# pkubioinformatics/nanoreviser

Measured on AMD Instinct MI355X. Metric: bases revised/sec (whole node), higher is better.
Workload: dtype f32 via scaled 2xf16 split (f32 accumulate)

## Files before the change

### nanoreviser_amd/csrc/nrv_api.hip

```cpp
#include "../../include/nanorev.h"
#include "nrv_kernels.h"
#include "nrv_tailfit.h"
#include "nrv_block.h"

#include <algorithm>
#include <cmath>
#include <cstdio>
#include <cstdlib>
#include <cstring>
#include <string>
#include <chrono>
#include <vector>

using namespace nrv;

#ifdef NRV_DEV_FAST
#define NRV_ACT1(...)
#else
#define NRV_ACT1(...) __VA_ARGS__
#endif

namespace {

thread_local std::string g_create_error = "";
// ... 689 lines not shown
            if (sc > 0 && sw > 0) { const double l = (room / sc - std::fabs((double)c0u[24 + o])) / sw; if (l < xl) xl = l; }
          }
          e2[24] = (float)(xl > 0 ? xl : 0.0);
        }
        d.cr_ep = put(e2, 25);
        const float* Wd = b.t(32);
        std::vector<uint16_t> df((size_t)13 * 4 * 2 * 512, 0);
        NRV_FOR (int ks = 0; ks < 13; ++ks)
          NRV_FOR (int mt = 0; mt < 4; ++mt)
            NRV_FOR (int lane = 0; lane < 64; ++lane)
              NRV_FOR (int j = 0; j < 8; ++j) {
                const int m = lane & 15, kg = lane >> 4;
                const int pos = 4 * ks + 2 * (j >> 2) + (kg >> 1), ch = 4 * (kg & 1) + (j & 3);
                const float v = pos < 50 ? std::ldexp(Wd[(size_t)(pos * 8 + ch) * 64 + 16 * mt + m], 10) : 0.f;
                const size_t o = ((size_t)((ks * 4 + mt) * 2) * 64 + lane) * 8 + j;
                split_f16(v, &df[o], &df[o + 512]);
              }
        std::vector<float> d2(df.size() / 2);
        memcpy(d2.data(), df.data(), df.size() * 2);
        d.cr_d = put(d2.data(), d2.size());
      }
      const float* c0 = host.data() + d.conv;
      memcpy(d.cr_k.w1, c0, 24 * 4);
      memcpy(d.cr_k.b1, c0 + 24, 8 * 4);
      NRV_FOR (int o = 0; o < 8; ++o) { d.cr_k.s1[o] = std::ldexp(c0[32 + o], 6); d.cr_k.h1[o] = std::ldexp(c0[40 + o], 6); }
    }
    const int K0[4] = {0, 32, 128, 256}, K1[4] = {0, 0, 64, 0}, s0[4] = {0, sX1, sX2, sX3}, s1[4] = {0, 0, sS, 0};
    const std::vector<float>* osc[4] = {nullptr, &sc2, &sc3, nullptr};
    const std::vector<float>* osh[4] = {nullptr, &sh2, &sh3, nullptr};
    const int sout[4] = {0, sX2, sX3, 13};
    d.hsc = pack_head_h2(b, wp, bs);
    d.h_w2 = put(wp.data(), wp.size());
    d.h_b2 = put(bs.data(), bs.size());
    NRV_FOR (int l = 1; l < 4; ++l) {
      const int E = plan_exponent(b, lbase[l], K0[l], s0[l], K1[l], s1[l], lH[l]);
      if (l == 1) {
        pack_lstm2_t(b, lbase[1], sX1, E, wp, bs);
        d.l2t_w = put(wp.data(), wp.size());
        d.l2t_b = put(bs.data(), bs.size());
      }
      if (l >= 2) {
        const int Kf = l == 2 ? 128 : 256;
        const std::vector<float>& fsc = l == 2 ? sc2 : sc3;
        const std::vector<float>& fsh = l == 2 ? sh2 : sh3;
        std::vector<float> all(b.p, b.p + b.off.back() + (size_t)C);
        NRV_FOR (int dir = 0; dir < 2; ++dir) {
          float* W = all.data() + b.off[lbase[l] + dir * 3 + 0];
          float* B = all.data() + b.off[lbase[l] + dir * 3 + 2];
          const int N4 = 4 * lH[l];
          NRV_FOR (int c = 0; c < N4; ++c) {
            double acc = B[c];
            NRV_FOR (int k = 0; k < Kf; ++k) acc += (double)fsh[k] * (double)W[(size_t)k * N4 + c];
            B[c] = (float)acc;
          }
          NRV_FOR (int k = 0; k < Kf; ++k)
            NRV_FOR (int c = 0; c < N4; ++c) W[(size_t)k * N4 + c] *= fsc[k];
        }
        const Blob bf{all.data(), b.off};
        const int Ef = plan_exponent(bf, lbase[l], K0[l], 13, K1[l], s1[l], lH[l]);
        pack_lstm_h2s(bf, lbase[l], K0[l], 13, K1[l], s1[l], lH[l], Ef, wp, bs, kUhS[l]);
        d.l_w2sf[l] = put(wp.data(), wp.size());
        d.l_b2sf[l] = put(bs.data(), bs.size());
        d.descale_f[l] = std::ldexp(1.f, -Ef);
      }
      d.descale[l] = std::ldexp(1.f, -E);
      std::vector<float> one(2 * lH[l], 1.f), zero(2 * lH[l], 0.f);
      d.l_s2[l] = put_scaled(osc[l] ? *osc[l] : one, sout[l] - 13);
      d.l_h2[l] = put_scaled(osh[l] ? *osh[l] : zero, sout[l]);
    }
  }
  pack_lstm1_16(b, 12, wp, bs);
  d.l1w16 = put(wp.data(), wp.size());
  d.l1b16 = put(bs.data(), bs.size());
  pack_dense(b.t(50), 128, 128, wp); d.d1p = put(wp.data(), wp.size());
  d.d1b = put(b.t(51), 128);
  pack_dense(b.t(52), 128, 32, wp); d.d2p = put(wp.data(), wp.size());
  d.d2b = put(b.t(53), 32);
  pack_dense(b.t(54), 32, 6, wp); d.mop = put(wp.data(), wp.size());
  {
    float mb[32] = {0};
    memcpy(mb, b.t(55), 6 * 4);
    d.mob = put(mb, 32);
  }
  pack_head_split(b, wp, bs);
  d.h_ws = put(wp.data(), wp.size());
  d.h_wb = put(bs.data(), bs.size());
  d.fw = put(b.t(56), (size_t)6 * T * 16);
  {
    std::vector<float> f8((size_t)16 * T * 8, 0.f);
    const float* fwp = b.t(56);
    NRV_FOR (int f = 0; f < 16; ++f)
      NRV_FOR (int t = 0; t < T; ++t)
        NRV_FOR (int k = 0; k < 6; ++k) f8[((size_t)f * T + t) * 8 + k] = fwp[(size_t)(t * 6 + k) * 16 + f];
    d.fw8 = put(f8.data(), f8.size());
  }
  d.fb = put(b.t(57), 16);
  d.ow = put(b.t(58), (size_t)16 * C);
  d.ob = put(b.t(59), C);
  d.n = host.size();
  HIPCHK(h, hipMalloc(&d.all, d.n * sizeof(float)));
  HIPCHK(h, hipMemcpy(d.all, host.data(), d.n * sizeof(float), hipMemcpyHostToDevice));
  return NRV_OK;
}

static void free_workspace(nrv_handle* h) {
  for (int m = 0; m < 2; ++m) {
    (void)hipFree(h->S[m]); (void)hipFree(h->X1[m]); (void)hipFree(h->X2[m]); (void)hipFree(h->X3[m]);
    (void)hipFree(h->MO[m]); h->MO[m] = nullptr;
    for (int st = 0; st < 2; ++st) { h->d_p[st][m] = nullptr; h->d_a[st][m] = nullptr; }
    h->S[m] = h->X1[m] = h->X2[m] = h->X3[m] = nullptr;
  }
  for (int st = 0; st < 2; ++st) {
    (void)hipFree(h->d_out[st]);
    h->d_out[st] = nullptr; h->d_sat_st[st] = nullptr; h->pin_sat[st] = nullptr; h->sat_seen[st] = 0;
    (void)hipHostFree(h->pin_out[st]);
    h->pin_out[st] = nullptr;
  }
  for (int st = 0; st < nrv_handle::kIn; ++st) {
    (void)hipFree(h->d_sig[st]); (void)hipFree(h->d_feat[st]);
    h->d_sig[st] = h->d_feat[st] = nullptr;
    (void)hipHostFree(h->pin_sig[st]); (void)hipHostFree(h->pin_feat[st]);
    h->pin_sig[st] = h->pin_feat[st] = nullptr;
  }
  h->pin_sig_cap = h->pin_feat_cap = 0;
  h->cap_rows = 0;
}

constexpr int kCoalesce = 4096;
static int group_windows(const nrv_handle* h) { return (h->coalesce && h->batch < kCoalesce) ? kCoalesce : h->batch; }

static int lanes_wanted(const nrv_handle* h) {
  if (h->coalesce) return 0;
  if (!h->lanes_on || h->batch > 2048 || h->batch % 32) return 0;
  const int w = 4096 / h->batch;
  return w > nrv_handle::kMaxLanes ? nrv_handle::kMaxLanes : w;
}
constexpr int kReadStageGroups = 4;
static int read_stage_groups(const nrv_handle* h) {
  static const int env = getenv("NRV_READ_STAGE") ? atoi(getenv("NRV_READ_STAGE")) : kReadStageGroups;
  return (lanes_wanted(h) > 1 || env < 1) ? 1 : (env > 8 ? 8 : env);
}
static int stage_windows(const nrv_handle* h, bool read_mode = false) {
  const int w = lanes_wanted(h);
  if (w > 1) return w * h->batch;
  return read_mode ? read_stage_groups(h) * group_windows(h) : group_windows(h);
}

static int ensure_workspace(nrv_handle* h) {
  const int T = h->T;
  const int rows = ((stage_windows(h, true) + kRowPad - 1) / kRowPad) * kRowPad;
  if (rows <= h->cap_rows) return NRV_OK;
  free_workspace(h);
  int rc;
  const size_t tiles = (size_t)(((group_windows(h) + kRowPad - 1) / kRowPad) * kRowPad) / 32;
  for (int m = 0; m < 2; ++m) {
    size_t nS = (tiles * T + 2) * 16 * 128, n1 = tiles * T * 8 * 128, n2 = tiles * T * 32 * 128,
           n3 = tiles * T * 64 * 128;
    HIPCHK(h, hipMalloc(&h->S[m], nS * 4));
    HIPCHK(h, hipMalloc(&h->X1[m], n1 * 4));
    HIPCHK(h, hipMalloc(&h->X2[m], n2 * 4));
    HIPCHK(h, hipMalloc(&h->X3[m], n3 * 4));
    HIPCHK(h, hipMalloc(&h->MO[m], tiles * T * 256 * 4));
    const size_t nm = tiles * T * 256;
    if ((rc = alloc_fill(h, h->MO[m], nm * 4)) || (rc = alloc_fill(h, h->S[m], nS * 4)) || (rc = alloc_fill(h, h->X1[m], n1 * 4)) ||
        (rc = alloc_fill(h, h->X2[m], n2 * 4)) || (rc = alloc_fill(h, h->X3[m], n3 * 4)))
      return rc;
    if (m == 0) { h->act_n[0] = nS; h->act_n[1] = n1; h->act_n[2] = n2; h->act_n[3] = n3; h->act_n[4] = nm; }
  }
  h->sig_bytes = (size_t)rows * T * kSig * 4 + 4096;
  h->feat_bytes = (size_t)rows * T * kFeat * 4 + 4096;
  for (int st = 0; st < nrv_handle::kIn; ++st) {
    HIPCHK(h, hipMalloc(&h->d_sig[st], h->sig_bytes));
    HIPCHK(h, hipMalloc(&h->d_feat[st], h->feat_bytes));
    if ((rc = poison_fill(h, h->d_sig[st], h->sig_bytes, nullptr)) || (rc = poison_fill(h, h->d_feat[st], h->feat_bytes, nullptr)))
      return rc;
  }
  for (int st = 0; st < 2; ++st) {
    const size_t ob = (size_t)rows * kOutBytes;
    HIPCHK(h, hipMalloc((void**)&h->d_out[st], ob + 64));
    HIPCHK(h, hipMemset(h->d_out[st], 0, ob + 64));
    if ((rc = poison_fill(h, h->d_out[st] + 64, ob, nullptr))) return rc;
    HIPCHK(h, hipHostMalloc((void**)&h->pin_out[st], ob + 64, hipHostMallocDefault));
    memset(h->pin_out[st], 0, ob + 64);
    h->d_p[st][0] = (float*)(h->d_out[st] + 64);
    h->d_p[st][1] = (float*)(h->d_out[st] + 64 + (size_t)rows * 24);
    h->d_a[st][0] = (int8_t*)(h->d_out[st] + 64 + (size_t)rows * 44);
    h->d_a[st][1] = (int8_t*)(h->d_out[st] + 64 + (size_t)rows * 45);
    h->d_sat_st[st] = (unsigned*)h->d_out[st];
    h->pin_sat[st] = (unsigned*)h->pin_out[st];
    h->sat_seen[st] = 0;
  }
  if (h->poison_on) HIPCHK(h, hipDeviceSynchronize());
  h->cap_rows = rows;
  return NRV_OK;
}

static void free_lanes(nrv_handle* h) {
  for (int l = 0; l < nrv_handle::kMaxLanes; ++l) {
    nrv_handle::Lane& L = h->lanes[l];
    if (L.stream) (void)hipStreamSynchronize(L.stream);
    for (int m = 0; m < 2; ++m) {
      (void)hipFree(L.S[m]); (void)hipFree(L.X1[m]); (void)hipFree(L.X2[m]); (void)hipFree(L.X3[m]); (void)hipFree(L.MO[m]);
      L.S[m] = L.X1[m] = L.X2[m] = L.X3[m] = L.MO[m] = nullptr;
    }
  }
  h->n_lanes = 0;
  h->lane_rows = 0;
}

static int ensure_lanes(nrv_handle* h) {
  const int T = h->T;
  const int rows = ((h->batch + kRowPad - 1) / kRowPad) * kRowPad;
  const int want = lanes_wanted(h);
  if (want == h->n_lanes && (want == 0 || rows <= h->lane_rows)) return NRV_OK;
  free_lanes(h);
  if (want == 0) return NRV_OK;
  const size_t tiles = rows / 32;
  const size_t nS = (tiles * T + 2) * 16 * 128, n1 = tiles * T * 8 * 128, n2 = tiles * T * 32 * 128,
               n3 = tiles * T * 64 * 128, nm = tiles * T * 256;
  if (!h->ev_fork) HIPCHK(h, hipEventCreateWithFlags(&h->ev_fork, hipEventDisableTiming));
  for (int l = 0; l < want; ++l) {
    nrv_handle::Lane& L = h->lanes[l];
    if (!L.stream) HIPCHK(h, hipStreamCreateWithFlags(&L.stream, hipStreamNonBlocking));
    if (!L.done) HIPCHK(h, hipEventCreateWithFlags(&L.done, hipEventDisableTiming));
    for (int m = 0; m < 2; ++m) {
      float** bufs[5] = {&L.S[m], &L.X1[m], &L.X2[m], &L.X3[m], &L.MO[m]};
      const size_t sz[5] = {nS, n1, n2, n3, nm};
      for (int i = 0; i < 5; ++i) {
        HIPCHK(h, hipMalloc(bufs[i], sz[i] * 4));
        const int rc = alloc_fill(h, *bufs[i], sz[i] * 4);
        if (rc) return rc;
        L.act_n[i] = sz[i];
      }
    }
  }
  HIPCHK(h, hipDeviceSynchronize());
  h->n_lanes = want;
  h->lane_rows = rows;
  return NRV_OK;
}

template <int KQ0, int KQ1, int H, int R, int WR>
static void launch_lstm_f32(nrv_handle* h, const LstmArgs& a, int tiles) {
  constexpr int NG = (H + 31) / 32;
  static_assert(NG * WR <= 4, "at most 4 waves per workgroup (one per SIMD, 512 registers each)");
#ifdef NRV_DEV_FAST
  return;
#else
  LstmArgs la = a;
  la.n_blk = (tiles + R * WR - 1) / (R * WR);
  dim3 grid(lstm_grid(la.n_blk)), blk(64 * NG * WR);
  if (h->act == 0) hipLaunchKernelGGL((lstm_layer_kernel<KQ0, KQ1, H, R, WR, false, 0>), grid, blk, 0, h->stream, la);
  NRV_ACT1(else hipLaunchKernelGGL((lstm_layer_kernel<KQ0, KQ1, H, R, WR, false, 1>), grid, blk, 0, h->stream, la);)
#endif
}


template <int KQ0, int KQ1, int H, int R, int WR>
static void launch_lstm_split(nrv_handle* h, const LstmArgs& a, const float* const ws[2], int tiles) {
  constexpr int NG = (H + 31) / 32;
#ifdef NRV_DEV_FAST
  return;
#else
  LstmSplitArgs sa;
  sa.T = a.T; sa.n_rows = a.n_rows;
  for (int m = 0; m < 2; ++m)
    sa.m[m] = LstmSplitModelParams{ws[m], a.m[m].bias, a.m[m].bn_scale, a.m[m].bn_shift, a.m[m].in0, a.m[m].in1,
                                   a.m[m].out};
  sa.n_blk = (tiles + R * WR - 1) / (R * WR);
  dim3 grid(lstm_grid(sa.n_blk)), blk(64 * NG * WR);
  if constexpr (R == 1) {
    {
      if (h->act == 0) hipLaunchKernelGGL((lstm_pair_kernel<KQ0, KQ1, H, R, WR, 0>), grid, blk, 0, h->stream, sa);
      NRV_ACT1(else hipLaunchKernelGGL((lstm_pair_kernel<KQ0, KQ1, H, R, WR, 1>), grid, blk, 0, h->stream, sa);)
      return;
    }
  }
  if constexpr (R != 1)
  {
    if (h->act == 0) hipLaunchKernelGGL((lstm_split_kernel<KQ0, KQ1, H, R, WR, 0>), grid, blk, 0, h->stream, sa);
    NRV_ACT1(else hipLaunchKernelGGL((lstm_split_kernel<KQ0, KQ1, H, R, WR, 1>), grid, blk, 0, h->stream, sa);)
  }
#endif
}

template <int KQ0, int KQ1, int H, int R, int WR, int UH, int NBG, int NA, int KBL = 0, bool RAW = false>
static void launch_lstm_h2s(nrv_handle* h, int layer, const ActView (&in0)[2], const ActView (&in1)[2],
                            float* const out[2], int T, int n, int tiles) {
  constexpr int NG = H / (16 * UH);
  LstmH2Args sa;
  sa.T = T; sa.n_rows = n;
  for (int m = 0; m < 2; ++m) {
    const DevModel& d = h->dm[m];
    sa.m[m] = LstmH2ModelParams{d.all + d.l_w2sf[layer], d.all + d.l_b2sf[layer],
                                d.all + d.l_s2[layer], d.all + d.l_h2[layer], in0[m], in1[m], out[m],
                                d.descale_f[layer]};
  }
  sa.n_blk = (tiles + R * WR - 1) / (R * WR);
  dim3 grid(lstm_grid(sa.n_blk)), blk(64 * NG * WR);
  if (h->act == 0) hipLaunchKernelGGL((lstm_h2s_kernel<KQ0, KQ1, H, R, WR, UH, 0, NBG, NA, KBL, RAW>), grid, blk, 0, h->stream, sa);
  NRV_ACT1(else hipLaunchKernelGGL((lstm_h2s_kernel<KQ0, KQ1, H, R, WR, UH, 1, NBG, NA, KBL, RAW>), grid, blk, 0, h->stream, sa);)
}

#ifndef NRV_L3_WS_NBG
#define NRV_L3_WS_NBG 4
#endif
template <int KQ0, int KQ1, int H>
static void launch_lstm_h2w(nrv_handle* h, int layer, const ActView (&in0)[2], const ActView (&in1)[2],
                            float* const out[2], int T, int n, int tiles) {
  LstmH2Args sa;
  sa.T = T; sa.n_rows = n;
  for (int m = 0; m < 2; ++m) {
    const DevModel& d = h->dm[m];
    sa.m[m] = LstmH2ModelParams{d.all + d.l_w2sf[layer], d.all + d.l_b2sf[layer], d.all + d.l_s2[layer], d.all + d.l_h2[layer],
                                in0[m], in1[m], out[m], d.descale_f[layer]};
  }
  sa.n_blk = (tiles + 1) / 2;
  dim3 grid(lstm_grid(sa.n_blk)), blk(512);
  if (h->act == 0) hipLaunchKernelGGL((lstm_h2w_kernel<KQ0, KQ1, H, 0, NRV_L3_WS_NBG>), grid, blk, 0, h->stream, sa);
  NRV_ACT1(else hipLaunchKernelGGL((lstm_h2w_kernel<KQ0, KQ1, H, 1, NRV_L3_WS_NBG>), grid, blk, 0, h->stream, sa);)
}

#if NRV_STAMP
static int g_only_stage = -1;
#define NRV_RUN_STAGE(k) (g_only_stage < 0 || g_only_stage == (k))
#else
#define NRV_RUN_STAGE(k) true
#endif

static int run_group(nrv_handle* h, const float* d_sig, const float* d_feat, int n, bool read_mode,
                     float* d_p1, float* d_p2, int8_t* d_a1, int8_t* d_a2, unsigned* sat) {
  const int T = h->T;
  const int tiles = (n + 31) / 32;
  if (h->poison_on) {
    for (int m = 0; m < 2; ++m) {
      float* const bufs[5] = {h->S[m], h->X1[m], h->X2[m], h->X3[m], h->MO[m]};
      for (int i = 0; i < 5; ++i) {
        const int rc0 = poison_fill(h, bufs[i], h->act_n[i] * 4, h->stream);
        if (rc0) return rc0;
      }
    }
  }
  hipEvent_t* ev = nullptr;
  if (h->prof && (h->prof != 3 || (h->prof_tick++ & 7) == 0)) {
    if (h->ev_used + NRV_N_KERNELS + 1 > h->ev_pool.size()) {
      for (int i = 0; i < NRV_N_KERNELS + 1; ++i) {
        hipEvent_t e;
        HIPCHK(h, hipEventCreate(&e));
        h->ev_pool.push_back(e);
      }
    }
    ev = h->ev_pool.data() + h->ev_used;
    h->ev_used += NRV_N_KERNELS + 1;
    if (h->prof == 1) HIPCHK(h, hipEventRecord(ev[0], h->stream));
  }
  auto mark = [&](int k) -> int {
    if (ev && (h->prof == 1 || k == 3 || k == 4)) HIPCHK(h, hipEventRecord(ev[k], h->stream));
    return NRV_OK;
  };
  int rc;

  bool h2_fused_l1 = false;
  {
    const int n_rows = read_mode ? n + T - 1 : n, Tc = read_mode ? 1 : T;
    const int n_tiles = read_mode ? (n + T - 1 + 31) / 32 : tiles * T;
    const int blocks = n_tiles < 128 ? n_tiles : 128;
    if (h->h2) {
      CnnRArgs a2;
      for (int m = 0; m < 2; ++m) {
        const DevModel& d = h->dm[m];
        a2.m[m] = CnnRModelParams{d.all + d.cr_w2, d.all + d.cr_ep, d.all + d.cr_d, d.all + d.cr_dbias, h->S[m]};
        a2.k[m] = d.cr_k;
      }
      a2.signal = d_sig; a2.T = Tc; a2.n_rows = n_rows; a2.n_tiles = n_tiles; a2.sat = sat;
      a2.l1_T = T; a2.l1_rows = n;
      for (int m = 0; m < 2; ++m) {
        const DevModel& d = h->dm[m];
        a2.l1[m] = Lstm1ModelParams{d.all + d.l1w16, d.all + d.l1b16, d.all + d.l1s2, d.all + d.l1h2, d_feat,
                                    read_mode ? 1 : 0, h->X1[m]};
      }
      const int wg_c = (2 * n_tiles + kCnnRWaves - 1) / kCnnRWaves, wg_l = (2 * ((n + 15) / 16) + kCnnRL1Waves - 1) / kCnnRL1Waves;
      const int wg = wg_c > wg_l ? wg_c : wg_l;
      if (!NRV_RUN_STAGE(0)) {}
      else if (h->act == 0) hipLaunchKernelGGL(cnn_r_kernel<0>, dim3(wg < 128 ? wg : 128, 2), dim3(kCnnRThreads), 0, h->stream, a2);
      NRV_ACT1(else hipLaunchKernelGGL(cnn_r_kernel<1>, dim3(wg < 128 ? wg : 128, 2), dim3(kCnnRThreads), 0, h->stream, a2);)
      h2_fused_l1 = true;
    } else {
      CnnArgs a;
      for (int m = 0; m < 2; ++m) {
        const DevModel& d = h->dm[m];
        a.m[m] = CnnModelParams{d.all + d.conv, d.all + d.dpack, d.all + d.dbias, d.all + d.dsplit, h->S[m]};
      }
      a.signal = d_sig; a.T = Tc; a.n_rows = n_rows; a.n_tiles = n_tiles;
#ifndef NRV_DEV_FAST
      if (h->split & 32) hipLaunchKernelGGL(cnn_kernel<true>, dim3(blocks, 2), dim3(kCnnThreads), 0, h->stream, a);
      else hipLaunchKernelGGL(cnn_kernel<false>, dim3(blocks, 2), dim3(kCnnThreads), 0, h->stream, a);
#endif
    }
    if ((rc = mark(1))) return rc;
  }
  auto win_view = [&](const float* p, int kq) { return ActView{p, kq, 0, T, 1}; };
  {
    LstmArgs a;
    a.T = T; a.n_rows = n;
    if (!h2_fused_l1) {
      Lstm1Args a1;
      a1.T = T; a1.n_rows = n;
      for (int m = 0; m < 2; ++m) {
        const DevModel& d = h->dm[m];
        a1.m[m] = Lstm1ModelParams{d.all + d.l1w16, d.all + d.l1b16, d.all + (h->h2 ? d.l1s2 : d.l_s[0]),
                                   d.all + (h->h2 ? d.l1h2 : d.l_h[0]), d_feat, read_mode ? 1 : 0, h->X1[m]};
      }
      dim3 grid((n + 63) / 64, 2, 2);
      if (h->h2) {
        if (h->act == 0) hipLaunchKernelGGL((lstm1_kernel<0, true>), grid, dim3(256), 0, h->stream, a1);
        NRV_ACT1(else hipLaunchKernelGGL((lstm1_kernel<1, true>), grid, dim3(256), 0, h->stream, a1);)
      } else if (h->act == 0) hipLaunchKernelGGL(lstm1_kernel<0>, grid, dim3(256), 0, h->stream, a1);
      NRV_ACT1(else hipLaunchKernelGGL(lstm1_kernel<1>, grid, dim3(256), 0, h->stream, a1);)
    }
    if ((rc = mark(2))) return rc;
    for (int m = 0; m < 2; ++m) {
      const DevModel& d = h->dm[m];
      a.m[m] = LstmModelParams{d.all + d.l_w[1], d.all + d.l_b[1], d.all + d.l_s[1], d.all + d.l_h[1],
                               win_view(h->X1[m], 8), ActView{}, nullptr, 0, h->X2[m]};
    }
    const ActView none[2] = {ActView{}, ActView{}};
    if (h->h2) {
      Lstm2RArgs ta;
      ta.T = T; ta.n_rows = n;
      for (int m = 0; m < 2; ++m) {
        const DevModel& d = h->dm[m];
        ta.m[m] = Lstm2RModelParams{d.all + d.l2t_w, d.all + d.l2t_b, h->X1[m], h->X2[m], d.descale[1]};
      }
      dim3 grid(2 * ((n + 63) / 64), 2, 2);
      if (!NRV_RUN_STAGE(2)) {}
      else if (h->act == 0) hipLaunchKernelGGL(lstm2_r_kernel<0>, grid, dim3(kL2rThreads), 0, h->stream, ta);
      NRV_ACT1(else hipLaunchKernelGGL(lstm2_r_kernel<1>, grid, dim3(kL2rThreads), 0, h->stream, ta);)
    }
    else if (h->split & 2) {
      const float* ws[2] = {h->dm[0].all + h->dm[0].l_ws[1], h->dm[1].all + h->dm[1].l_ws[1]};
      launch_lstm_split<8, 0, 64, 1, 2>(h, a, ws, tiles);
    } else {
      launch_lstm_f32<8, 0, 64, 1, 2>(h, a, tiles);
    }
    if ((rc = mark(3))) return rc;
    for (int m = 0; m < 2; ++m) {
      const DevModel& d = h->dm[m];
      ActView sv = read_mode ? ActView{h->S[m], 16, 1, 1, 0} : win_view(h->S[m], 16);
      a.m[m] = LstmModelParams{d.all + d.l_w[2], d.all + d.l_b[2], d.all + d.l_s[2], d.all + d.l_h[2],
                               win_view(h->X2[m], 32), sv, nullptr, 0, h->X3[m]};
    }
    if (h->h2) {
      const ActView i0[2] = {win_view(h->X2[0], 32), win_view(h->X2[1], 32)};
      const ActView i1[2] = {read_mode ? ActView{h->S[0], 16, 1, 1, 0} : win_view(h->S[0], 16),
                             read_mode ? ActView{h->S[1], 16, 1, 1, 0} : win_view(h->S[1], 16)};
      float* const o[2] = {h->X3[0], h->X3[1]};
      if (NRV_RUN_STAGE(3)) launch_lstm_h2w<32, 16, 128>(h, 2, i0, i1, o, T, n, tiles);
    } else if (h->split & 4) {
      const float* ws[2] = {h->dm[0].all + h->dm[0].l_ws[2], h->dm[1].all + h->dm[1].l_ws[2]};
      launch_lstm_split<32, 16, 128, 2, 1>(h, a, ws, tiles);
    } else {
      launch_lstm_f32<32, 16, 128, 1, 1>(h, a, tiles);
    }
    if ((rc = mark(4))) return rc;
    for (int m = 0; m < 2; ++m) {
      const DevModel& d = h->dm[m];
      a.m[m] = LstmModelParams{d.all + d.l_w[3], d.all + d.l_b[3], d.all + d.l_s[3], d.all + d.l_h[3],
                               win_view(h->X3[m], 64), ActView{}, nullptr, 0, h->X2[m] };
    }
    if (h->h2) {
      const ActView i0[2] = {win_view(h->X3[0], 64), win_view(h->X3[1], 64)};
      float* const o[2] = {h->X2[0], h->X2[1]};
      if (NRV_RUN_STAGE(4)) launch_lstm_h2s<64, 0, 64, 2, 1, 1, 8, 2, 3, true>(h, 3, i0, none, o, T, n, tiles);
    } else if (h->split & 8) {
      const float* ws[2] = {h->dm[0].all + h->dm[0].l_ws[3], h->dm[1].all + h->dm[1].l_ws[3]};
      launch_lstm_split<64, 0, 64, 1, 2>(h, a, ws, tiles);
    } else {
      launch_lstm_f32<64, 0, 64, 1, 2>(h, a, tiles);
    }
    if ((rc = mark(5))) return rc;
  }
  {
    float* dp[2] = {d_p1 ? d_p1 : h->d_p[0][0], d_p2 ? d_p2 : h->d_p[0][1]};
    int8_t* da[2] = {d_a1 ? d_a1 : h->d_a[0][0], d_a2 ? d_a2 : h->d_a[0][1]};
    if (h->h2) {
      HeadH2Args ha;
      ha.T = T; ha.n_rows = n; ha.n_tiles = tiles;
      for (int m = 0; m < 2; ++m) {
        const DevModel& d = h->dm[m];
        ha.m[m] = HeadH2ModelParams{d.all + d.h_w2, d.all + d.h_b2, h->X2[m], d.all + d.fw8, d.all + d.fb, d.all + d.ow,
                                    d.all + d.ob, dp[m], da[m], d.hsc.c12, d.hsc.c23, d.hsc.c3o, d.C};
      }
      if (NRV_RUN_STAGE(5)) hipLaunchKernelGGL(head_h2_kernel, dim3(tiles < 128 ? tiles : 128, 2), dim3(kHeadH2Threads), 0, h->stream, ha);
      if ((rc = mark(6))) return rc;
      HIPCHK(h, hipGetLastError());
      return NRV_OK;
    }
    HeadArgs a;
    a.T = T; a.n_rows = n;
    for (int m = 0; m < 2; ++m) {
      const DevModel& d = h->dm[m];
      a.m[m] = HeadModelParams{d.all + d.d1p, d.all + d.d1b, d.all + d.d2p, d.all + d.d2b,
                               d.all + d.mop, d.all + d.mob, d.all + d.fw, d.all + d.fb,
                               d.all + d.ow, d.all + d.ob, h->X2[m], h->MO[m], dp[m], da[m], d.C};
    }
    if (h->split & 16) {
      HeadSplitArgs sa;
      sa.n_units = tiles * T;
      for (int m = 0; m < 2; ++m) {
        const DevModel& d = h->dm[m];
        sa.m[m] = HeadSplitModelParams{d.all + d.h_ws, d.all + d.h_wb, h->X2[m], h->MO[m]};
      }
      const int blocks = sa.n_units < 512 ? (sa.n_units + 3) / 4 : 128;
#ifndef NRV_DEV_FAST
      hipLaunchKernelGGL(head_mlp_split_kernel, dim3(blocks, 2), dim3(256), 0, h->stream, sa);
    } else {
      hipLaunchKernelGGL(head_mlp_kernel, dim3(tiles * T, 2), dim3(64), 0, h->stream, a);
#endif
    }
#ifndef NRV_DEV_FAST
    hipLaunchKernelGGL(head_final_kernel, dim3(tiles, 2), dim3(256), 0, h->stream, a);
#endif
    if ((rc = mark(6))) return rc;
  }
  HIPCHK(h, hipGetLastError());
  return NRV_OK;
}

static int prof_collect(nrv_handle* h) {
  if (h->ev_used == 0) return NRV_OK;
  HIPCHK(h, hipStreamSynchronize(h->stream));
  for (size_t g = 0; g + NRV_N_KERNELS + 1 <= h->ev_used; g += NRV_N_KERNELS + 1)
    for (int k = 0; k < NRV_N_KERNELS; ++k) {
      if (h->prof != 1 && k != 3) continue;
      float ms = 0.f;
      HIPCHK(h, hipEventElapsedTime(&ms, h->ev_pool[g + k], h->ev_pool[g + k + 1]));
      h->prof_ms[k] += ms;
      h->prof_n[k] += 1;
    }
  h->ev_used = 0;
  return NRV_OK;
}

static int check_handle(nrv_handle* h) {
  if (!h) return NRV_E_INVALID;
  hipError_t e = hipSetDevice(h->device);
  if (e != hipSuccess) { h->err = std::string("hipSetDevice: ") + hipGetErrorString(e); return NRV_E_HIP; }
  return NRV_OK;
}

}

extern "C" {

int nrv_create(const nrv_weights* m1, const nrv_weights* m2, int T, int device, int recurrent_act,
               nrv_handle** out) {
  if (!out) { g_create_error = "nrv_create: out is NULL"; return NRV_E_INVALID; }
  *out = nullptr;
  if (T < 1 || T > kMaxT) { g_create_error = "nrv_create: window length T out of range [1,32]"; return NRV_E_INVALID; }
  if (recurrent_act != 0 && recurrent_act != 1) { g_create_error = "nrv_create: recurrent_act must be 0 or 1"; return NRV_E_INVALID; }
  Blob b1, b2;
  if (!make_blob(m1, T, 6, &b1)) { g_create_error = "nrv_create: model1 blob size does not match the graph for this T (expect 6 classes)"; return NRV_E_WEIGHTS; }
  if (!make_blob(m2, T, 5, &b2)) { g_create_error = "nrv_create: model2 blob size does not match the graph for this T (expect 5 classes)"; return NRV_E_WEIGHTS; }
  int ndev = 0;
  hipError_t e = hipGetDeviceCount(&ndev);
  if (e != hipSuccess || ndev <= 0) {
    g_create_error = std::string("nrv_create: no HIP device (") + hipGetErrorString(e) + "); this library has no CPU fallback";
    return NRV_E_NO_DEVICE;
  }
  if (device < 0 || device >= ndev) { g_create_error = "nrv_create: device index out of range"; return NRV_E_NO_DEVICE; }
  e = hipSetDevice(device);
  if (e != hipSuccess) { g_create_error = std::string("hipSetDevice: ") + hipGetErrorString(e); return NRV_E_HIP; }
  nrv_handle* h = new (std::nothrow) nrv_handle();
  if (!h) { g_create_error = "out of host memory"; return NRV_E_NOMEM; }
  h->device = device; h->T = T; h->act = recurrent_act;
  if (const char* s = getenv("NRV_PRECISION")) {
    if (!strcmp(s, "f32")) { h->split = 0; h->h2 = 0; }
    else if (!strcmp(s, "bf16x3")) { h->split = 62; h->h2 = 0; }
    else if (!strcmp(s, "f16x2")) { h->split = 62; h->h2 = 1; }
  }
  int rc = NRV_OK;
  e = hipStreamCreateWithFlags(&h->own_stream, hipStreamDefault);
  if (e != hipSuccess) { g_create_error = std::string("hipStreamCreate: ") + hipGetErrorString(e); delete h; return NRV_E_HIP; }
  h->stream = h->own_stream;
  bool ok = hipStreamCreateWithFlags(&h->copy_stream, hipStreamNonBlocking) == hipSuccess &&
            hipStreamCreateWithFlags(&h->d2h_stream, hipStreamNonBlocking) == hipSuccess;
  for (int st = 0; st < nrv_handle::kIn && ok; ++st) ok = hipEventCreateWithFlags(&h->ev_in[st], hipEventDisableTiming) == hipSuccess;
  for (int st = 0; st < 2 && ok; ++st)
    ok = hipEventCreateWithFlags(&h->ev_done[st], hipEventDisableTiming) == hipSuccess &&
         hipEventCreateWithFlags(&h->ev_out[st], hipEventDisableTiming) == hipSuccess;
  if (const char* e2 = getenv("NRV_HOST_REGISTER")) h->host_register = atoi(e2) != 0;
  if (const char* e3 = getenv("NRV_LANES")) h->lanes_on = atoi(e3) != 0;
  if (const char* e4 = getenv("NRV_COALESCE")) h->coalesce = atoi(e4) != 0;
  if (const char* e6 = getenv("NRV_LABELS_BUDGET"); e6 && *e6) { const long long v = atoll(e6); if (v > 0) h->lab_budget = (size_t)v; }
  if (const char* e7 = getenv("NRV_FIT_MAX_ROWS"); e7 && *e7) { const long long v = atoll(e7); if (v > 0) h->fit.max_rows = v > ((long long)1 << 31) - 1 ? ((long long)1 << 31) - 1 : v; }
  if (const char* e5 = getenv("NRV_POISON"); e5 && *e5) { h->poison_on = true; h->poison = (unsigned)strtoul(e5, nullptr, 16); }
  ok = ok && hipMalloc((void**)&h->d_sat, 4 * sizeof(unsigned)) == hipSuccess &&
       hipMemset(h->d_sat, 0, 4 * sizeof(unsigned)) == hipSuccess;
  if (!ok) { g_create_error = "nrv_create: could not create the copy stream / events / counters"; nrv_destroy(h); return NRV_E_HIP; }
  if ((rc = upload_model(h, 0, b1, 6)) || (rc = upload_model(h, 1, b2, 5)) || (rc = ensure_workspace(h))) {
    g_create_error = h->err;
    nrv_destroy(h);
    return rc;
  }
  *out = h;
  return NRV_OK;
}

void nrv_destroy(nrv_handle* h) {
  if (!h) return;
  (void)hipSetDevice(h->device);
  if (h->stream) (void)hipStreamSynchronize(h->stream);
  free_workspace(h);
  free_lanes(h);
  for (int l = 0; l < nrv_handle::kMaxLanes; ++l) {
    if (h->lanes[l].done) (void)hipEventDestroy(h->lanes[l].done);
    if (h->lanes[l].stream) (void)hipStreamDestroy(h->lanes[l].stream);
  }
  if (h->ev_fork) (void)hipEventDestroy(h->ev_fork);
  for (int m = 0; m < 2; ++m) (void)hipFree(h->dm[m].all);
  for (hipEvent_t e : h->ev_pool) (void)hipEventDestroy(e);
  if (h->copy_stream) { (void)hipStreamSynchronize(h->copy_stream); (void)hipStreamDestroy(h->copy_stream); }
  if (h->d2h_stream) { (void)hipStreamSynchronize(h->d2h_stream); (void)hipStreamDestroy(h->d2h_stream); }
  if (h->edit_stream) { (void)hipStreamSynchronize(h->edit_stream); (void)hipStreamDestroy(h->edit_stream); }
  if (h->lab_stream) { (void)hipStreamSynchronize(h->lab_stream); (void)hipStreamDestroy(h->lab_stream); }
  (void)hipFree(h->d_lab);
  for (char* p : h->lab_retired) (void)hipFree(p);
  for (int m = 0; m < 2; ++m) {
    (void)hipFree(h->fit.flat[m]); (void)hipFree(h->fit.y[m]);
    (void)hipFree(h->fit.m[m].d_par); (void)hipFree(h->fit.m[m].d_state); (void)hipFree(h->fit.m[m].d_lr);
  }
  (void)hipFree(h->fit.d_partial); (void)hipFree(h->fit.d_pstat); (void)hipFree(h->fit.d_order); (void)hipFree(h->fit.d_p);
  for (int st = 0; st < nrv_handle::kIn; ++st) if (h->ev_in[st]) (void)hipEventDestroy(h->ev_in[st]);
  for (int st = 0; st < 2; ++st) {
    if (h->ev_done[st]) (void)hipEventDestroy(h->ev_done[st]);
    if (h->ev_out[st]) (void)hipEventDestroy(h->ev_out[st]);
  }
  (void)hipFree(h->d_raw); (void)hipFree(h->d_starts); (void)hipFree(h->d_reads);
  for (auto& sl : h->raw_slot) {
    (void)hipFree(sl.d_in); (void)hipFree(sl.d_out); (void)hipHostFree(sl.pin_in); (void)hipHostFree(sl.pin_out);
    (void)hipFree(sl.d_stat);
    (void)hipFree(sl.d_mrg); (void)hipHostFree(sl.pin_mrg);
    if (sl.ev_in) (void)hipEventDestroy(sl.ev_in);
    if (sl.ev_done) (void)hipEventDestroy(sl.ev_done);
    if (sl.ev_out) (void)hipEventDestroy(sl.ev_out);
  }
  (void)hipFree(h->d_sat);
  if (h->ev_raw) (void)hipEventDestroy(h->ev_raw);
  if (h->own_stream) (void)hipStreamDestroy(h->own_stream);
  delete h;
}

int nrv_set_batch(nrv_handle* h, int batch) {
  int rc = check_handle(h);
  if (rc) return rc;
  if (batch < 1 || batch > (1 << 20)) { h->err = "nrv_set_batch: batch out of range"; return NRV_E_INVALID; }
  HIPCHK(h, hipStreamSynchronize(h->stream));
  h->batch = batch;
  if ((rc = ensure_workspace(h))) return rc;
  return ensure_lanes(h);
}
int nrv_get_batch(nrv_handle* h) { return h ? h->batch : NRV_E_INVALID; }

int nrv_set_precision(nrv_handle* h, int mode) {
  int rc = check_handle(h);
  if (rc) return rc;
  if (mode != NRV_PREC_F32 && mode != NRV_PREC_BF16X3 && mode != NRV_PREC_F16X2) {
    h->err = "nrv_set_precision: unknown mode";
    return NRV_E_INVALID;
  }
  h->split = mode == NRV_PREC_F32 ? 0 : 62;
  h->h2 = mode == NRV_PREC_F16X2;
  return NRV_OK;
}
int nrv_get_precision(nrv_handle* h) {
  if (!h) return NRV_E_INVALID;
  return h->h2 ? NRV_PREC_F16X2 : (h->split ? NRV_PREC_BF16X3 : NRV_PREC_F32);
}

int nrv_set_stream(nrv_handle* h, void* s) {
  int rc = check_handle(h);
  if (rc) return rc;
  HIPCHK(h, hipStreamSynchronize(h->stream));
  h->stream = s ? (hipStream_t)s : h->own_stream;
  return NRV_OK;
}

int nrv_sync(nrv_handle* h) {
  int rc = check_handle(h);
  if (rc) return rc;
  HIPCHK(h, hipStreamSynchronize(h->stream));
  return NRV_OK;
}

}

template <class F>
static int for_groups(nrv_handle* h, int64_t n, F&& body) {
  const int64_t G = group_windows(h);
  const int64_t ng = (n + G - 1) / G;
  int nl = (h->n_lanes > 1 && ng > 1 && h->prof == 0) ? h->n_lanes : 0;
  if ((int64_t)nl > ng) nl = (int)ng;
  hipStream_t main = h->stream;
  float* keep[5][2];
  for (int m = 0; m < 2; ++m) { keep[0][m] = h->S[m]; keep[1][m] = h->X1[m]; keep[2][m] = h->X2[m]; keep[3][m] = h->X3[m]; keep[4][m] = h->MO[m]; }
  size_t keep_n[5];
  memcpy(keep_n, h->act_n, sizeof keep_n);
  auto restore = [&]() {
    for (int m = 0; m < 2; ++m) { h->S[m] = keep[0][m]; h->X1[m] = keep[1][m]; h->X2[m] = keep[2][m]; h->X3[m] = keep[3][m]; h->MO[m] = keep[4][m]; }
    memcpy(h->act_n, keep_n, sizeof keep_n);
    h->stream = main;
  };
  if (nl) {
    HIPCHK(h, hipEventRecord(h->ev_fork, main));
    for (int l = 0; l < nl; ++l) HIPCHK(h, hipStreamWaitEvent(h->lanes[l].stream, h->ev_fork, 0));
  }
  int rc = NRV_OK;
  int64_t g = 0;
  for (int64_t s = 0; s < n && !rc; s += G, ++g) {
    const int nb = (int)((n - s < G) ? (n - s) : G);
    if (nl) {
      const nrv_handle::Lane& L = h->lanes[g % nl];
      for (int m = 0; m < 2; ++m) { h->S[m] = L.S[m]; h->X1[m] = L.X1[m]; h->X2[m] = L.X2[m]; h->X3[m] = L.X3[m]; h->MO[m] = L.MO[m]; }
      memcpy(h->act_n, L.act_n, sizeof L.act_n);
      h->stream = L.stream;
    }
    rc = body(s, nb);
  }
  restore();
  if (nl) {
    for (int l = 0; l < nl; ++l) {
      hipError_t e = hipEventRecord(h->lanes[l].done, h->lanes[l].stream);
      if (e == hipSuccess) e = hipStreamWaitEvent(main, h->lanes[l].done, 0);
      if (e != hipSuccess && !rc) { h->err = std::string("lane join: ") + hipGetErrorString(e); rc = NRV_E_HIP; }
    }
  }
  return rc;
}

template <class Begin>
static int begin_then_end(nrv_handle* h, Begin begin) {
  int t = -1;
  const int rc = begin(&t);
  return rc ? rc : nrv_reads_raw_end(h, t);
}
template <class Fetch>
static int merged_collect(nrv_handle* h, const char* who, const char* who_edits, const char* head, const MergeView& v,
                          const MergeLayout& m, const MergeOut& o, bool want_q, size_t blob_cap, Fetch fetch) {
  const int64_t n = v.N - h->T > 0 ? v.N - h->T : 0;
  const size_t nb = ((size_t)v.n_reads + 1) * 8;
  const int64_t total = ((const int64_t*)head)[v.n_reads];
  if (total < 0 || total > v.N + n) { h->err = std::string(who) + ": merged block out of range"; return NRV_E_HIP; }
  memcpy(o.off, head, nb);
  if (o.seq) memcpy(o.seq, head + m.seq, (size_t)total);
  if (want_q && o.qual) memcpy(o.qual, head + m.qual, (size_t)total);
  if (o.report) memcpy(o.report, head + m.rep, (size_t)v.n_reads * kReportCols * 8);
  if (o.profile) memcpy(o.profile, head + m.prof, (size_t)v.n_reads * kProfileCols * 8);
  if (o.trim) memcpy(o.trim, head + m.trim, (size_t)v.n_reads * 16);
  if (o.accuracy) memcpy(o.accuracy, head + m.accu, (size_t)v.n_reads * kAccuracyCols * 8);
  if (o.errclass) memcpy(o.errclass, head + m.ecls, (size_t)v.n_reads * kErrclassCols * 8);
  if (o.infix) memcpy(o.infix, head + m.infx, (size_t)v.n_reads * kInfixCols * 8);
  if (o.score) memcpy(o.score, head + m.scor, (size_t)v.n_reads * kScoreCols * 8);
  int rc = NRV_OK;
  if (o.edit_off) {
    const int64_t n_ed = ((const int64_t*)(head + m.eoff))[v.n_reads];
    if (n_ed < 0 || n_ed > n) { h->err = std::string(who_edits) + ": edit list out of range"; return NRV_E_HIP; }
    memcpy(o.edit_off, head + m.eoff, nb);
    if (n_ed > 0 && (rc = fetch(o.edits, m.edits, (size_t)n_ed * sizeof(nrv_edit)))) return rc;
  }
  if (o.rec_off) {
    const int64_t n_b = ((const int64_t*)(head + m.roff))[v.n_reads];
    if (n_b < 0 || (uint64_t)n_b > blob_cap) { h->err = std::string(who) + ": records out of range"; return NRV_E_HIP; }
    memcpy(o.rec_off, head + m.roff, nb);
    if (n_b > 0 && (rc = fetch(o.blob, m.blob, (size_t)n_b))) return rc;
  }
  return NRV_OK;
// ... 2262 lines not shown
```

### nanoreviser_amd/csrc/nrv_kernels.h

```cpp
#pragma once
#include "nrv_common.h"
#include "nrv_cnn.h"
#include "nrv_lstm1.h"
#include "nrv_lstm_f32.h"
#include "nrv_lstm_bf16x3.h"
#include "nrv_lstm_f16x2.h"
#include "nrv_lstm_f16x2s.h"
#include "nrv_lstm_f16x2w.h"
#include "nrv_lstm2_u.h"
#include "nrv_cnn_r.h"
#include "nrv_head.h"
#include "nrv_head_f16x2.h"
#include "nrv_segment.h"
#include "nrv_stats.h"
#include "nrv_merge.h"
#include "nrv_report.h"
#include "nrv_edits.h"
#include "nrv_pack.h"
#include "nrv_profile.h"
#include "nrv_trim.h"
#include "nrv_align.h"
#include "nrv_errclass.h"
#include "nrv_infix.h"
#include "nrv_labels.h"
#include "nrv_score.h"
```

Measured before the change: 12.40 million.

## Add dedicated software-pipelined LSTM layer-4 kernel with resident recurrent weights

```diff
diff --git a/nanoreviser_amd/csrc/nrv_api.hip b/nanoreviser_amd/csrc/nrv_api.hip
--- a/nanoreviser_amd/csrc/nrv_api.hip
+++ b/nanoreviser_amd/csrc/nrv_api.hip
@@ -1015,6 +1015,20 @@
   NRV_ACT1(else hipLaunchKernelGGL((lstm_h2s_kernel<KQ0, KQ1, H, R, WR, UH, 1, NBG, NA, KBL, RAW>), grid, blk, 0, h->stream, sa);)
 }
 
+static void launch_lstm4_r(nrv_handle* h, int layer, const ActView (&in0)[2], float* const out[2], int T, int n, int tiles) {
+  LstmH2Args sa;
+  sa.T = T; sa.n_rows = n;
+  for (int m = 0; m < 2; ++m) {
+    const DevModel& d = h->dm[m];
+    sa.m[m] = LstmH2ModelParams{d.all + d.l_w2sf[layer], d.all + d.l_b2sf[layer], d.all + d.l_s2[layer], d.all + d.l_h2[layer],
+                                in0[m], ActView{}, out[m], d.descale_f[layer]};
+  }
+  sa.n_blk = (tiles + 1) / 2;
+  dim3 grid(lstm_grid(sa.n_blk)), blk(kL4rThreads);
+  if (h->act == 0) hipLaunchKernelGGL(lstm4_r_kernel<0>, grid, blk, 0, h->stream, sa);
+  NRV_ACT1(else hipLaunchKernelGGL(lstm4_r_kernel<1>, grid, blk, 0, h->stream, sa);)
+}
+
 #ifndef NRV_L3_WS_NBG
 #define NRV_L3_WS_NBG 4
 #endif
@@ -1184,7 +1198,11 @@
     if (h->h2) {
       const ActView i0[2] = {win_view(h->X3[0], 64), win_view(h->X3[1], 64)};
       float* const o[2] = {h->X2[0], h->X2[1]};
+#if defined(NRV_L4_H2S) || NRV_STAMP
       if (NRV_RUN_STAGE(4)) launch_lstm_h2s<64, 0, 64, 2, 1, 1, 8, 2, 3, true>(h, 3, i0, none, o, T, n, tiles);
+#else
+      if (NRV_RUN_STAGE(4)) launch_lstm4_r(h, 3, i0, o, T, n, tiles);
+#endif
     } else if (h->split & 8) {
       const float* ws[2] = {h->dm[0].all + h->dm[0].l_ws[3], h->dm[1].all + h->dm[1].l_ws[3]};
       launch_lstm_split<64, 0, 64, 1, 2>(h, a, ws, tiles);
diff --git a/nanoreviser_amd/csrc/nrv_kernels.h b/nanoreviser_amd/csrc/nrv_kernels.h
--- a/nanoreviser_amd/csrc/nrv_kernels.h
+++ b/nanoreviser_amd/csrc/nrv_kernels.h
@@ -6,6 +6,7 @@
 #include "nrv_lstm_bf16x3.h"
 #include "nrv_lstm_f16x2.h"
 #include "nrv_lstm_f16x2s.h"
+#include "nrv_lstm4_r.h"
 #include "nrv_lstm_f16x2w.h"
 #include "nrv_lstm2_u.h"
 #include "nrv_cnn_r.h"
diff --git a/nanoreviser_amd/csrc/nrv_lstm4_r.h b/nanoreviser_amd/csrc/nrv_lstm4_r.h
--- /dev/null
+++ b/nanoreviser_amd/csrc/nrv_lstm4_r.h
@@ -0,0 +1,336 @@
+#pragma once
+#include "nrv_lstm_f16x2s.h"
+
+namespace nrv {
+
+#ifndef NRV_L4_KBL
+#define NRV_L4_KBL 3
+#endif
+#ifndef NRV_L4_KBR
+#define NRV_L4_KBR 5
+#endif
+#ifndef NRV_L4_NBG
+#define NRV_L4_NBG 4
+#endif
+constexpr int kL4rThreads = 256;
+
+template <int ACT, int KBL = NRV_L4_KBL, int KBR = NRV_L4_KBR, int NBG = NRV_L4_NBG>
+__global__ void __launch_bounds__(kL4rThreads)
+lstm4_r_kernel(const LstmH2Args args) {
+  constexpr int H = 64, R = 2, NA = 2;
+  constexpr int NG = H / 16;
+  constexpr int KK_IN = 8, KK_REC = H / 32, KK = KK_IN + KK_REC;
+  constexpr int RT = 2 * R;
+  constexpr int EPK = 4, TPE = 3 * RT;
+  constexpr int ROWS = 32 * R;
+  constexpr int GS = ROWS * 8 + 8;
+  constexpr int TERM = (H / 8) * GS;
+  constexpr int HBUF = TERM;
+  constexpr int NTHREADS = kL4rThreads;
+  constexpr int LBG = NBG - 1, LA = NA - 1;
+  constexpr int NS = EPK * (KK - KBR);
+  constexpr int NRES = EPK * KBR;
+  static_assert(KBR >= KK_REC && KBL + KBR <= KK, "the recurrent blocks are resident; LDS and register blocks are disjoint");
+  static_assert(NS % NBG == 0 && LBG <= NS, "the ring must divide the entries it serves");
+  static_assert(NRES <= NS, "the resident entries are requested behind in(0)'s ring-served entries");
+
+  constexpr int NE = RT * 4;
+  __shared__ __attribute__((aligned(16))) float hbuf[2 * HBUF];
+  __shared__ __attribute__((aligned(16))) float wl[KBL > 0 ? NG * KBL * EPK * 512 : 4];
+
+  const int lane = threadIdx.x & 63;
+  const int wave = __builtin_amdgcn_readfirstlane(threadIdx.x >> 6);
+  const int hg = wave;
+  const int l15 = lane & 15, kq = lane >> 4;
+  const LstmBlock blk = lstm_block();
+  if (blk.rowblk >= args.n_blk) return;
+  const int dir = blk.dir;
+  const LstmH2ModelParams& P = args.m[blk.model];
+  const int T = args.T;
+  const int row0 = blk.rowblk * ROWS;
+
+  const __amdgpu_buffer_rsrc_t wrs = make_rsrc(
+      (const char*)P.wsplit + ((size_t)(dir * NG + hg) * KK) * (EPK * 2 * 1024), KK * EPK * 2 * 1024);
+  const unsigned wlane = lane * 16;
+  const float* bp = P.bias + (size_t)(dir * NG + hg) * 4 * 16 + l15;
+  const float dsc = P.descale, dsc02 = 0.2f * dsc, dsc2 = 2.885390081777927f * dsc;
+  const float bi = bp[0 * 16] * dsc, bf = bp[1 * 16] * dsc, bg = bp[2 * 16] * dsc, bo = bp[3 * 16] * dsc;
+  const float kI = __builtin_fmaf(bi, 0.2f, 0.5f), kF = __builtin_fmaf(bf, 0.2f, 0.5f), kO = __builtin_fmaf(bo, 0.2f, 0.5f),
+              kG = bg * 2.885390081777927f;
+  const int u0 = hg * 16 + l15;
+  const int hw_off = (u0 >> 3) * GS + (4 * kq) * 8 + (u0 & 7);
+  const int hp_off = kq * GS + l15 * 8;
+
+  float* const wlw = wl + (wave * KBL * EPK) * 512 + lane * 4;
+  if constexpr (KBL > 0) {
+#pragma unroll 1
+    for (int e0 = 0; e0 < KBL * EPK; e0 += 4) {
+      f32x4 v[8];
+#pragma unroll
+      for (int j = 0; j < 8; ++j) v[j] = buf_load16(wrs, wlane, ((e0 + j / 2) * 2 + (j & 1)) * 1024);
+#pragma unroll
+      for (int j = 0; j < 8; ++j) *(f32x4*)(wlw + ((e0 + j / 2) * 2 + (j & 1)) * 256) = v[j];
+    }
+  }
+  for (int i = threadIdx.x; i < HBUF; i += NTHREADS) hbuf[i] = 0.f;
+  float c[NE];
+#pragma unroll
+  for (int i = 0; i < NE; ++i) c[i] = 0.f;
+  __syncthreads();
+
+  struct ABase {
+    __amdgpu_buffer_rsrc_t r0[R];
+    unsigned v0[R][2];
+  };
+  auto mk_base = [&](int s) __attribute__((always_inline)) {
+    const int sc = s < T ? s : T - 1;
+    const int t = dir ? (T - 1 - sc) : sc;
+    ABase ab;
+#pragma unroll
+    for (int r = 0; r < R; ++r) {
+      ab.r0[r] = make_rsrc(P.in0.ubase(row0 + r * 32, t), 0xffffffffu);
+#pragma unroll
+      for (int sub = 0; sub < 2; ++sub)
+        ab.v0[r][sub] = (P.in0.voff(row0 + r * 32, t, l15 + 16 * sub, kq & 1) + (kq >> 1) * 512) * 4;
+    }
+    return ab;
+  };
+  struct BReg { f16x8 t[2]; };
+  struct AReg { f32x4 v[2]; };
+  BReg b[NBG];
+  BReg wres[NRES];
+  AReg a[NA][RT];
+  auto loadB = [&](int e, BReg& bb) __attribute__((always_inline)) {
+    if (e < KBL * EPK) {
+      bb.t[0] = __builtin_bit_cast(f16x8, *(const f32x4*)(wlw + (e * 2) * 256));
+      bb.t[1] = __builtin_bit_cast(f16x8, *(const f32x4*)(wlw + (e * 2 + 1) * 256));
+    } else {
+      bb.t[0] = __builtin_bit_cast(f16x8, buf_load16(wrs, wlane, (e * 2) * 1024));
+      bb.t[1] = __builtin_bit_cast(f16x8, buf_load16(wrs, wlane, (e * 2 + 1) * 1024));
+    }
+  };
+  auto loadA_in = [&](const ABase& ab, int kk, int rt, AReg& d) __attribute__((always_inline)) {
+    const int r = rt >> 1, sub = rt & 1;
+    d.v[1] = buf_load16(ab.r0[r], ab.v0[r][sub], kk * 4096 + 1024);
+    d.v[0] = buf_load16(ab.r0[r], ab.v0[r][sub], kk * 4096);
+  };
+  auto loadA_rec = [&](const _Float16* hp, int kkr, int rt, AReg& d) __attribute__((always_inline)) {
+    const _Float16* qh = hp + kkr * 4 * GS + rt * 128;
+    d.v[1] = *(const f32x4*)(qh + TERM);
+    d.v[0] = *(const f32x4*)(qh);
+  };
+  auto loadA_in1 = [&](const ABase& ab, int kk, int rt, int term, AReg& d) __attribute__((always_inline)) {
+    const int r = rt >> 1, sub = rt & 1;
+    d.v[term] = buf_load16(ab.r0[r], ab.v0[r][sub], kk * 4096 + term * 1024);
+  };
+  auto loadA_rec1 = [&](const _Float16* hp, int kkr, int rt, int term, AReg& d) __attribute__((always_inline)) {
+    d.v[term] = *(const f32x4*)(hp + kkr * 4 * GS + rt * 128 + term * TERM);
+  };
+  constexpr int APPE = (2 * RT + EPK - 1) / EPK;
+  static_assert(4 + APPE <= 3 * RT, "fragment pieces must fit behind an entry's products");
+  constexpr int PA[3] = {0, 1, 0}, PB[3] = {1, 0, 0};
+
+  constexpr int GST = 14;
+  struct GateSt { float zi, zf, zg, zo, cp, p, hv, t; _Float16 hh, hl; };
+  auto gate_stage = [&](GateSt& g, const f32x4 (&Z)[4][RT], _Float16* hw, int e, int st) __attribute__((always_inline)) {
+    const int rt = (e / 4) % RT, reg = e % 4;
+    if (st == 0) {
+      g.zi = Z[0][rt][reg]; g.zf = Z[1][rt][reg];
+      g.cp = c[e];
+    } else if (st == 1) {
+      g.zg = Z[2][rt][reg]; g.zo = Z[3][rt][reg];
+    } else if (st == 2) {
+      if constexpr (ACT == 0) {
+        g.zi = __builtin_fminf(__builtin_fmaxf(__builtin_fmaf(g.zi, dsc02, kI), 0.0f), 1.0f);
+        g.zf = __builtin_fminf(__builtin_fmaxf(__builtin_fmaf(g.zf, dsc02, kF), 0.0f), 1.0f);
+      } else {
+        g.zi = sigmoid_exact(__builtin_fmaf(g.zi, dsc, bi));
+        g.zf = sigmoid_exact(__builtin_fmaf(g.zf, dsc, bf));
+      }
+    } else if (st == 3) {
+      if constexpr (ACT == 0) g.zo = __builtin_fminf(__builtin_fmaxf(__builtin_fmaf(g.zo, dsc02, kO), 0.0f), 1.0f);
+      else g.zo = sigmoid_exact(__builtin_fmaf(g.zo, dsc, bo));
+      g.zg = __builtin_fmaf(g.zg, dsc2, kG);
+    } else if (st == 4) {
+      g.zg = __builtin_amdgcn_exp2f(g.zg);
+    } else if (st == 5) {
+      g.t = __builtin_amdgcn_rcpf(g.zg + 1.0f);
+    } else if (st == 6) {
+      g.p = g.zi * __builtin_fmaf(g.t, -2.0f, 1.0f);
+    } else if (st == 7) {
+      const float cn = __builtin_fmaf(g.zf, g.cp, g.p);
+      c[e] = cn;
+      g.zg = cn * 2.885390081777927f;
+    } else if (st == 8) {
+      g.zg = __builtin_amdgcn_exp2f(g.zg);
+    } else if (st == 9) {
+      g.t = __builtin_amdgcn_rcpf(g.zg + 1.0f);
+    } else if (st == 10) {
+      g.hv = g.zo * __builtin_fmaf(g.t, -2.0f * kHScale, kHScale);
+    } else if (st == 11) {
+      g.hh = (_Float16)g.hv;
+    } else if (st == 12) {
+      g.hl = (_Float16)(g.hv - (float)g.hh);
+    } else {
+      hw[(rt * 16 + reg) * 8] = g.hh;
+      hw[(rt * 16 + reg) * 8 + TERM] = g.hl;
+    }
+  };
+  constexpr int ITEMS = (H / 16) * 2 * ROWS;
+  constexpr int NIT = ITEMS / NTHREADS;
+  static_assert(ITEMS % NTHREADS == 0, "copy-out items must divide evenly");
+  constexpr int CST = 4;
+  struct CopySt { f16x8 hi, lo; float* dst; };
+  auto copy_stage = [&](CopySt& k, const _Float16* himg, int t, int i, int st) __attribute__((always_inline)) {
+    const int it = threadIdx.x + i * NTHREADS;
+    constexpr int KBH = H / 16;
+    const int kbh = it / ROWS, rr = it % ROWS;
+    if (st == 0) {
+      k.hi = *(const f16x8*)(himg + kbh * GS + rr * 8);
+      k.lo = *(const f16x8*)(himg + kbh * GS + rr * 8 + TERM);
+      const int tile = blk.rowblk * R + rr / 32;
+      k.dst = P.out + ((size_t)(tile * T + t) * (2 * H / 4) + (dir * KBH + (kbh >> 1)) * 4 + (kbh & 1)) * 128 + (rr & 31) * 4;
+    } else if (st == 1) {
+      *(f16x8*)k.dst = k.hi;
+    } else if (st == 2) {
+      *(f16x8*)(k.dst + 2 * 128) = k.lo;
+    }
+  };
+
+  constexpr int NTICK = KK_IN * EPK * TPE;
+  constexpr int NGP = NE * GST, NCP = NIT * CST;
+  constexpr int TG_WANT = NGP < (2 * NTICK) / 3 ? NGP : (2 * NTICK) / 3;
+  constexpr int TG_MAX = (KK_IN - LA) * EPK * TPE;
+  constexpr int TG = TG_WANT < TG_MAX ? TG_WANT : TG_MAX;
+  constexpr int TC = NTICK - TG;
+  static_assert(TG >= 1 && TC >= 1, "no room for the gates / copy-out in the input phase");
+  auto in_phase = [&](auto work_tag, f32x4 (&N)[4][RT], const f32x4 (&Z)[4][RT], const ABase& xb,
+                      const _Float16* hp_next, _Float16* himg_w, int t_out, const ABase& xb_wrap) __attribute__((always_inline)) {
+    constexpr bool WORK = decltype(work_tag)::value;
+    GateSt gs;
+    CopySt cs;
+#pragma unroll
+    for (int kk = 0; kk < KK_IN; ++kk) {
+      const int ka = kk + LA;
+#pragma unroll
+      for (int rt = 0; rt < RT; ++rt) {
+        if (ka < KK_IN) loadA_in(xb, ka, rt, a[ka % NA][rt]);
+        else if (WORK) loadA_rec(hp_next, ka - KK_IN, rt, a[ka % NA][rt]);
+        else loadA_in(xb_wrap, ka - KK_IN, rt, a[ka % NA][rt]);
+      }
+#pragma unroll
+      for (int ge = 0; ge < EPK; ++ge) {
+        const int e = EPK * kk + ge, g = ge;
+        if (e < NS) loadB((e + LBG) % NS, b[(e + LBG) % NBG]);
+        if (!WORK && e < NRES) {
+          wres[e].t[0] = __builtin_bit_cast(f16x8, buf_load16(wrs, wlane, ((NS + e) * 2) * 1024));
+          wres[e].t[1] = __builtin_bit_cast(f16x8, buf_load16(wrs, wlane, ((NS + e) * 2 + 1) * 1024));
+        }
+        __builtin_amdgcn_sched_barrier(0);
+        const BReg& be = e < NS ? b[e % NBG] : wres[e < NS ? 0 : e - NS];
+#pragma unroll
+        for (int rt = 0; rt < RT; ++rt)
+#pragma unroll
+          for (int pr = 0; pr < 3; ++pr) {
+            const int tk = (e * RT + rt) * 3 + pr;
+            N[g][rt] = mfma16_f16(__builtin_bit_cast(f16x8, a[kk % NA][rt].v[PA[pr]]), be.t[PB[pr]],
+                                  (kk == 0 && pr == 0) ? f32x4{0.f, 0.f, 0.f, 0.f} : N[g][rt]);
+            if constexpr (WORK) {
+              if (tk < TG) {
+#pragma unroll
+                for (int pc = (tk * NGP) / TG; pc < ((tk + 1) * NGP) / TG; ++pc)
+                  gate_stage(gs, Z, himg_w + hw_off, pc / GST, pc % GST);
+              } else {
+#pragma unroll
+                for (int pc = ((tk - TG) * NCP) / TC; pc < ((tk - TG + 1) * NCP) / TC; ++pc)
+                  copy_stage(cs, himg_w, t_out, pc / CST, pc % CST);
+              }
+              __builtin_amdgcn_sched_barrier(0);
+              if (tk == TG - 1) __syncthreads();
+            }
+          }
+        __builtin_amdgcn_sched_barrier(0);
+      }
+    }
+  };
+  auto rec_phase = [&](f32x4 (&Z)[4][RT], const _Float16* hp, const ABase& xb_next) __attribute__((always_inline)) {
+#pragma unroll
+    for (int kr = 0; kr < KK_REC; ++kr) {
+      const int kk = KK_IN + kr;
+      const int ka = kk + LA;
+#pragma unroll
+      for (int ge = 0; ge < EPK; ++ge) {
+        const int e = EPK * kk + ge, g = ge;
+        __builtin_amdgcn_sched_barrier(0);
+#pragma unroll
+        for (int rt = 0; rt < RT; ++rt)
+#pragma unroll
+          for (int pr = 0; pr < 3; ++pr) {
+            Z[g][rt] = mfma16_f16(__builtin_bit_cast(f16x8, a[kk % NA][rt].v[PA[pr]]), wres[e - NS].t[PB[pr]], Z[g][rt]);
+            const int m = rt * 3 + pr, pa = ge * APPE + (m - 4);
+            if (m >= 4 && m < 4 + APPE && pa < 2 * RT) {
+              __builtin_amdgcn_sched_barrier(0);
+              const int rn = pa / 2, tn = pa % 2;
+              if (ka < KK) loadA_rec1(hp, ka - KK_IN, rn, tn, a[ka % NA][rn]);
+              else loadA_in1(xb_next, ka - KK, rn, tn, a[ka % NA][rn]);
+              __builtin_amdgcn_sched_barrier(0);
+            }
+          }
+        __builtin_amdgcn_sched_barrier(0);
+      }
+    }
+  };
+
+  f32x4 Z[4][RT], N[4][RT];
+  auto himg = [&](int s) __attribute__((always_inline)) { return (_Float16*)(hbuf + ((s + 1) & 1) * HBUF); };
+  auto t_of = [&](int s) __attribute__((always_inline)) { return dir ? (T - 1 - s) : s; };
+
+  {
+    const ABase x0 = mk_base(0), x1 = mk_base(1);
+#pragma unroll
+    for (int e = 0; e < LBG; ++e) loadB(e, b[e]);
+#pragma unroll
+    for (int i = 0; i < LA; ++i)
+#pragma unroll
+      for (int rt = 0; rt < RT; ++rt) loadA_in(x0, i, rt, a[i][rt]);
+    in_phase(std::false_type{}, Z, Z, x0, nullptr, nullptr, 0, x1);
+  }
+#pragma unroll
+  for (int i = 0; i < NRES; ++i) {
+    asm volatile("" : "+a"(wres[i].t[0]));
+    asm volatile("" : "+a"(wres[i].t[1]));
+  }
+  auto last_step = [&](int s) __attribute__((always_inline)) {
+    GateSt gs;
+#pragma unroll
+    for (int e = 0; e < NE; ++e) {
+#pragma unroll
+      for (int st = 0; st < GST; ++st) gate_stage(gs, Z, himg(s) + hw_off, e, st);
+      if ((e & 3) == 3) __builtin_amdgcn_sched_barrier(0);
+    }
+    __syncthreads();
+    CopySt cs;
+#pragma unroll
+    for (int i = 0; i < NIT; ++i)
+#pragma unroll
+      for (int st = 0; st < CST; ++st) copy_stage(cs, himg(s), t_of(s), i, st);
+  };
+#pragma unroll 1
+  for (int s = 0; s + 1 < T; ++s) {
+    const ABase xn = mk_base(s + 1);
+    if (s > 0) rec_phase(Z, himg(s - 1) + hp_off, xn);
+    in_phase(std::true_type{}, N, Z, xn, himg(s) + hp_off, himg(s), t_of(s), xn);
+#pragma unroll
+    for (int g = 0; g < 4; ++g)
+#pragma unroll
+      for (int rt = 0; rt < RT; ++rt) Z[g][rt] = N[g][rt];
+  }
+  {
+    const int s = T - 1;
+    const ABase xn = mk_base(s + 1);
+    if (s > 0) rec_phase(Z, himg(s - 1) + hp_off, xn);
+    last_step(s);
+  }
+}
+
+}
```

Result: faster. 12.66 million, median of 6 (+2.1%).
